# amazon-science/glass-text-spotting

Measured on AMD Instinct MI355X. Metric: images/sec/GPU end-to-end spotting, 1000x1000, ~32 RoIs; 1/2/4/8 GPU scaling, higher is better.
Workload: dtype f32

## Files before the change

glass-text-spotting_amd/csrc/wino_common.h:

```cpp
#pragma once
#include "common.h"
#include <cstdint>
#include <cstdlib>
#include <type_traits>
#include <utility>

typedef float f32x16 __attribute__((ext_vector_type(16)));
typedef unsigned u32x4 __attribute__((ext_vector_type(4)));

namespace {

constexpr unsigned OOB = 0x7fffffffu;

struct WinoParams {
  const float* x;
  const float* u;
  const float* bias;
  const float* res;
  float* y;
  int N, H, W, Cin, Cout, TH, TW, ntiles, nk;
  int nkt;
  long y_slice;
  int ldx, ldy, ycoff, ldr, relu, res_mode;
  int tiles_m, tiles_n;
  unsigned x_bytes, u_bytes, y_bytes, r_bytes;
  unsigned magic_tpi, magic_tw;
  unsigned long long* dbg;
};

__device__ __forceinline__ float4 add4(float4 a, float4 b) { return make_float4(a.x + b.x, a.y + b.y, a.z + b.z, a.w + b.w); }
__device__ __forceinline__ float4 sub4(float4 a, float4 b) { return make_float4(a.x - b.x, a.y - b.y, a.z - b.z, a.w - b.w); }
__device__ __forceinline__ int fast_div(int t, int d, unsigned magic) {
  int q = d == 1 ? t : (int)__umulhi((unsigned)t, magic);
  if (t - q * d >= d) ++q;
  return q;
}

template <int I> using ic = std::integral_constant<int, I>;
template <int... Is, class F> __device__ __forceinline__ void static_for_impl(std::integer_sequence<int, Is...>, F&& f) {
  (f(ic<Is>{}), ...);
}
template <int N, class F> __device__ __forceinline__ void static_for(F&& f) {
  static_for_impl(std::make_integer_sequence<int, N>{}, static_cast<F&&>(f));
}

__device__ __forceinline__ float comp(const float4& v, int s) { return s == 0 ? v.x : s == 1 ? v.y : s == 2 ? v.z : v.w; }

}
```

glass-text-spotting_amd/csrc/winograd43.hip:

```cpp
#include "wino_common.h"
#include "splitk_common.h"
#include <vector>

typedef float f32x4 __attribute__((ext_vector_type(4)));
typedef float f32x2 __attribute__((ext_vector_type(2)));
typedef unsigned u32x2 __attribute__((ext_vector_type(2)));

namespace {

constexpr int WINO43_LDS_BYTES = 2 * 36 * 16 * 32 * 4;
#ifndef GLASS_W43_RING
#define GLASS_W43_RING 6
#endif
constexpr int RING = GLASS_W43_RING;
#ifndef GLASS_W43_VACC_XI
#define GLASS_W43_VACC_XI 32
#endif
#ifndef GLASS_W43_STORE_AUX
#define GLASS_W43_STORE_AUX 0
#endif
constexpr int W43_STORE_AUX = GLASS_W43_STORE_AUX;
constexpr int VACC_XI = GLASS_W43_VACC_XI;
constexpr unsigned INV = 0x40000000u;

// ... 46 lines not shown
  constexpr int K4 = KT;
  constexpr int V4_FLOATS = 36 * T4 * K4;
  constexpr int HALVES = KT / 16;
  constexpr int NG = 36 * HALVES;
  constexpr int SPG = 144 / NG;
  constexpr int SLOTS = KT / 4;
  constexpr int RPW = 64 / KT;
  static_assert(NG % RING == 0, "ring slot = group % RING must be consistent across k-tiles");
  extern __shared__ __attribute__((aligned(16))) float smem[];
  const int nblk = gridDim.x, bid = blockIdx.x;
  const int xcd = bid & 7, q8 = nblk >> 3, r8 = nblk & 7;
  const int logical = (xcd < r8 ? xcd * (q8 + 1) : r8 * (q8 + 1) + (xcd - r8) * q8) + (bid >> 3);
  const int tile_m = logical / p.tiles_n;
  const int tile_n = logical - tile_m * p.tiles_n;
  const int t0 = tile_m * T4, n0 = tile_n * N4;

  const int tid = threadIdx.x, lane = tid & 63;
  const int wv = __builtin_amdgcn_readfirstlane(tid >> 6);
  const int tpi = p.TH * p.TW;
  const int kt0 = blockIdx.y * p.nk;
  const int xk0 = kt0 * (KT * 4), uk0 = tile_n * p.nkt + kt0;
  unsigned long long stamp0 = 0, stamp1 = 0, stamp2 = 0, real0 = 0;
  if constexpr (ABL == 4) { stamp0 = __builtin_amdgcn_s_memtime(); real0 = __builtin_amdgcn_s_memrealtime(); }

  __amdgpu_buffer_rsrc_t xr = __builtin_amdgcn_make_buffer_rsrc(const_cast<float*>(p.x), 0, (int)p.x_bytes, 0x00020000);
  __amdgpu_buffer_rsrc_t ur = __builtin_amdgcn_make_buffer_rsrc(const_cast<float*>(p.u), 0, (int)p.u_bytes, 0x00020000);

  const int c2 = tid % (KT / 2), tl = tid / (KT / 2);
  const int wc = WC == 4 ? wv : (wv & (WC - 1)), wt = WC == 4 ? 0 : (wv / WC);
  unsigned rowoff[6], coloff[6];
  {
    const int t = t0 + tl;
    const bool tv = t < p.ntiles;
    const int n = fast_div(t, tpi, p.magic_tpi);
    const int rem = t - n * tpi;
    const int th = fast_div(rem, p.TW, p.magic_tw);
    const int tw = rem - th * p.TW;
    const int h0 = 4 * th - 1, w0 = 4 * tw - 1;
#pragma unroll
    for (int r = 0; r < 6; ++r) {
      const int hi = h0 + r;
      rowoff[r] = (tv && (unsigned)hi < (unsigned)p.H) ? (unsigned)(((n * p.H + hi) * p.W) * p.ldx * 4) : INV;
    }
#pragma unroll
    for (int c = 0; c < 6; ++c) {
      const int wi = w0 + c;
      coloff[c] = ((unsigned)wi < (unsigned)p.W) ? (unsigned)((wi * p.ldx + 2 * c2) * 4) : INV;
    }
  }
  f32x2 dd[36];
  auto load_patch1 = [&](int kt, auto i_) {
    constexpr int i = decltype(i_)::value;
    if constexpr (ABL == 3) { if (kt > 1) return; }
    dd[i] = __builtin_bit_cast(f32x2, __builtin_amdgcn_raw_buffer_load_b64(xr, rowoff[i / 6] + coloff[i % 6], xk0 + kt * (K4 * 4), 0));
  };
  float* vdst = smem + tl * K4 + (((c2 >> 1) ^ ((tl / RPW) % SLOTS)) * 4) + (c2 & 1) * 2;
  Bt6p bt;
  auto row_step = [&](auto c_, auto s_) {
    constexpr int c = decltype(c_)::value, S = decltype(s_)::value;
    if constexpr (ABL == 2) return;
    bt.template step<S>(dd[0 + c], dd[6 + c], dd[12 + c], dd[18 + c], dd[24 + c], dd[30 + c]);
    if constexpr (S == 5) {
      dd[0 + c] = bt.o0; dd[6 + c] = bt.o1; dd[12 + c] = bt.o2; dd[18 + c] = bt.o3; dd[24 + c] = bt.o4; dd[30 + c] = bt.o5;
    }
  };
  auto vstore = [&](int stage, int xi, f32x2 v) {
    *reinterpret_cast<f32x2*>(vdst + stage * V4_FLOATS + xi * (T4 * K4)) = v;
  };
  auto col_step = [&](int stage, auto i_, auto s_) {
    constexpr int i = decltype(i_)::value, S = decltype(s_)::value;
    if constexpr (ABL == 2) {
      if constexpr (S == 1) vstore(stage, i * 6 + 0, dd[i * 6 + 0]);
      if constexpr (S == 2) vstore(stage, i * 6 + 1, dd[i * 6 + 1]);
      if constexpr (S == 3) vstore(stage, i * 6 + 2, dd[i * 6 + 2]);
      if constexpr (S == 4) vstore(stage, i * 6 + 5, dd[i * 6 + 5]);
      if constexpr (S == 5) { vstore(stage, i * 6 + 3, dd[i * 6 + 3]); vstore(stage, i * 6 + 4, dd[i * 6 + 4]); }
      return;
    }
    bt.template step<S>(dd[i * 6 + 0], dd[i * 6 + 1], dd[i * 6 + 2], dd[i * 6 + 3], dd[i * 6 + 4], dd[i * 6 + 5]);
    if constexpr (S == 1) vstore(stage, i * 6 + 0, bt.o0);
// ... 74 lines not shown
        }
        if constexpr (xi >= VACC_XI) {
          f32x4 c = acc[xi][cb];
          const float af = comp4(aq[u % RING][cb], s), bf = comp4(vq[u & 1], s);
          asm volatile("v_mfma_f32_16x16x4_f32 %0, %1, %2, %0" : "+v"(c) : "v"(af), "v"(bf));
          acc[xi][cb] = c;
        } else {
          acc[xi][cb] = __builtin_amdgcn_mfma_f32_16x16x4f32(comp4(aq[u % RING][cb], s), comp4(vq[u & 1], s), acc[xi][cb], 0, 0, 0);
        }
      });
      __builtin_amdgcn_sched_barrier(0);
    });
    __syncthreads();
  }

  if constexpr (VACC_XI < 36) {
    asm volatile("s_nop 15\n\ts_nop 15" ::: "memory");
#pragma unroll
    for (int i = VACC_XI; i < 36; ++i) {
      asm volatile("" : "+v"(acc[i][0]));
      asm volatile("" : "+v"(acc[i][1]));
    }
  }
  if constexpr (ABL == 4) stamp2 = __builtin_amdgcn_s_memtime();
  __amdgpu_buffer_rsrc_t yr = __builtin_amdgcn_make_buffer_rsrc(p.y + (long)blockIdx.y * p.y_slice, 0, (int)p.y_bytes, 0x00020000);
  __amdgpu_buffer_rsrc_t rr = __builtin_amdgcn_make_buffer_rsrc(const_cast<float*>(p.res_mode == 1 ? p.res : p.y), 0,
                                                                 (int)(p.res_mode == 1 ? p.r_bytes : 0u), 0x00020000);
  const int cbase = n0 + 32 * wc + 4 * kg;
  const unsigned ldy4 = (unsigned)p.ldy * 4u, ldr4 = (unsigned)p.ldr * 4u;
  unsigned yrow[4], ycol[4], rrow[4], rcol[4];
  {
    const int t = t0 + vt;
    const bool tv = t < p.ntiles;
    const int n = fast_div(t, tpi, p.magic_tpi);
    const int rem = t - n * tpi;
    const int th = fast_div(rem, p.TW, p.magic_tw);
    const int tw = rem - th * p.TW;
    const unsigned pix = (unsigned)((n * p.H + 4 * th) * p.W + 4 * tw);
#pragma unroll
    for (int a = 0; a < 4; ++a) {
      const bool ok = tv && 4 * th + a < p.H;
      yrow[a] = ok ? (pix + (unsigned)(a * p.W)) * ldy4 + (unsigned)(p.ycoff + cbase) * 4u : INV;
      rrow[a] = ok ? (pix + (unsigned)(a * p.W)) * ldr4 + (unsigned)cbase * 4u : INV;
    }
#pragma unroll
    for (int b = 0; b < 4; ++b) {
      const bool ok = 4 * tw + b < p.W;
      ycol[b] = ok ? (unsigned)b * ldy4 : INV;
      rcol[b] = ok ? (unsigned)b * ldr4 : INV;
    }
  }
  const float lo2 = p.relu == 2 ? 0.f : __builtin_nanf(""), lo1 = p.relu == 1 ? 0.f : __builtin_nanf("");
  f32x4 rres[2][16];
  auto load_res = [&](auto cb_) {
    constexpr int cb = decltype(cb_)::value;
    if (p.res_mode == 1) {
#pragma unroll
      for (int a = 0; a < 4; ++a)
#pragma unroll
        for (int b = 0; b < 4; ++b)
          rres[cb][a * 4 + b] = __builtin_bit_cast(f32x4, __builtin_amdgcn_raw_buffer_load_b128(rr, rrow[a] + rcol[b], cb * 64, 0));
    }
  };
#ifdef GLASS_W43_SPLIT_STORES
  load_res(ic<0>{});
  static_for<2>([&](auto cb_) {
    constexpr int cb = decltype(cb_)::value;
    f32x4 bv = f32x4{0.f, 0.f, 0.f, 0.f};
    if (p.bias != nullptr) bv = *reinterpret_cast<const f32x4*>(p.bias + cbase + 16 * cb);
    f32x4 out[16];
#pragma unroll
    for (int e = 0; e < 4; ++e) {
      float z[6][4];
#pragma unroll
      for (int i = 0; i < 6; ++i)
        at4(acc[i * 6 + 0][cb][e], acc[i * 6 + 1][cb][e], acc[i * 6 + 2][cb][e], acc[i * 6 + 3][cb][e], acc[i * 6 + 4][cb][e],
            acc[i * 6 + 5][cb][e], z[i][0], z[i][1], z[i][2], z[i][3]);
#pragma unroll
      for (int b = 0; b < 4; ++b) {
        float y0, y1, y2, y3;
        at4(z[0][b], z[1][b], z[2][b], z[3][b], z[4][b], z[5][b], y0, y1, y2, y3);
        out[0 * 4 + b][e] = y0; out[1 * 4 + b][e] = y1; out[2 * 4 + b][e] = y2; out[3 * 4 + b][e] = y3;
// ... 97 lines not shown
}

}

static bool wino43_wide(int Cout, int Cin) { return Cout % 128 == 0 && Cin % 32 == 0; }

extern "C" int glass_winograd43_supported(const glass_conv_desc* d) {
  if (!d) return 0;
  const long xb = (long)d->N * d->H * d->W * d->ldx * 4;
  const long yb = (long)d->N * d->H * d->W * d->ldy * 4, rb = d->res_mode == 1 ? (long)d->N * d->H * d->W * d->ldr * 4 : 0;
  const long lim = 0x40000000L;
  return d->KH == 3 && d->KW == 3 && d->stride_h == 1 && d->stride_w == 1 && d->pad_h == 1 && d->pad_w == 1 &&
         d->Cin % 16 == 0 && d->Cout % 64 == 0 && d->ldx % 2 == 0 && d->ldx >= d->Cin && d->y_cstride == 1 && d->ldy % 4 == 0 &&
         d->y_coff % 4 == 0 && d->y_coff >= 0 && d->y_coff + d->Cout <= d->ldy &&
         (d->res_mode == 0 || (d->res_mode == 1 && d->ldr % 4 == 0 && d->ldr >= d->Cout)) && xb < lim && yb < lim && rb < lim &&
         36L * d->Cout * d->Cin * 4 < 0x7fffff00L && d->Ho == d->H && d->Wo == d->W;
}

extern "C" size_t glass_winograd43_weight_floats(int Cout, int Cin) { return (size_t)36 * (size_t)Cout * (size_t)Cin; }

extern "C" int glass_winograd43_pack_weights(const float* w, int Cout, int Cin, float* u_packed, glass_stream_t stream) {
  GLASS_CHECK_ARG(w && u_packed, "glass_winograd43_pack_weights: null pointer");
  GLASS_CHECK_ARG(Cout > 0 && Cin > 0 && Cout % 64 == 0 && Cin % 16 == 0,
                  "glass_winograd43_pack_weights: Cout=%d must be a multiple of 64 and Cin=%d a multiple of 16", Cout, Cin);
  const long total = 36L * Cout * Cin;
  const int blocks = (int)((total + 255) / 256 < 8192 ? (total + 255) / 256 : 8192);
  const bool wide = wino43_wide(Cout, Cin);
  hipLaunchKernelGGL(wino43_pack_weights_kernel, dim3(blocks), dim3(256), 0, (hipStream_t)stream, w, u_packed, Cout, Cin,
                     wide ? 4 : 2, wide ? 32 : 16);
  GLASS_CHECK_LAUNCH("glass_winograd43_pack_weights");
  return GLASS_OK;
}

static int wino43_launch(const glass_conv_desc* d, const float* x, const float* u_packed, const float* bias, const float* residual,
                         float* y, glass_stream_t stream, bool body_only, int splits = 1, void* workspace = nullptr);

extern "C" int glass_conv3x3_winograd43_nhwc(const glass_conv_desc* d, const float* x, const float* u_packed,
                                             const float* bias, const float* residual, float* y, glass_stream_t stream) {
  return wino43_launch(d, x, u_packed, bias, residual, y, stream, false);
}

extern "C" int glass_conv3x3_winograd43_body_nhwc(const glass_conv_desc* d, const float* x, const float* u_packed,
                                                  const float* bias, const float* residual, float* y, glass_stream_t stream) {
  GLASS_CHECK_ARG(d && d->W >= 4, "glass_conv3x3_winograd43_body_nhwc: needs W >= 4");
  return wino43_launch(d, x, u_packed, bias, residual, y, stream, true);
}

extern "C" int glass_winograd43_splitk_supported(const glass_conv_desc* d, int splits) {
  return glass_winograd43_supported(d) && wino43_wide(d->Cout, d->Cin) && splits >= 2 && splits <= 32 && (d->Cin / 32) % splits == 0 &&
         (long)d->N * d->H * d->W * d->Cout * 4 < 0x40000000L;
}

extern "C" int64_t glass_winograd43_splitk_workspace_bytes(const glass_conv_desc* d, int splits) {
  if (!d) return 0;
  return (int64_t)splits * d->N * d->H * d->W * d->Cout * (int64_t)sizeof(float);
}

extern "C" int glass_conv3x3_winograd43_splitk_nhwc(const glass_conv_desc* d, const float* x, const float* u_packed, const float* bias,
                                                    const float* residual, float* y, int splits, int body_only, void* workspace,
                                                    int64_t workspace_bytes, glass_stream_t stream) {
  GLASS_CHECK_ARG(d && workspace, "glass_conv3x3_winograd43_splitk_nhwc: null pointer");
  GLASS_CHECK_ARG(glass_winograd43_splitk_supported(d, splits),
                  "glass_conv3x3_winograd43_splitk_nhwc: needs the wide F(4x4) shape (Cout %% 128 == 0, Cin %% 32 == 0), 2 <= splits <= 32 "
                  "dividing Cin / 32 (got Cin=%d Cout=%d splits=%d)", d->Cin, d->Cout, splits);
  GLASS_CHECK_ARG(workspace_bytes >= glass_winograd43_splitk_workspace_bytes(d, splits) && ((uintptr_t)workspace & 15) == 0,
                  "glass_conv3x3_winograd43_splitk_nhwc: workspace too small or not 16-byte aligned");
  GLASS_CHECK_ARG(!body_only || d->W >= 4, "glass_conv3x3_winograd43_splitk_nhwc: body_only needs W >= 4");
  return wino43_launch(d, x, u_packed, bias, residual, y, stream, body_only != 0, splits, workspace);
}

static int wino43_launch(const glass_conv_desc* d, const float* x, const float* u_packed, const float* bias, const float* residual,
                         float* y, glass_stream_t stream, bool body_only, int splits, void* workspace) {
  GLASS_CHECK_ARG(d && x && u_packed && y, "glass_conv3x3_winograd43_nhwc: null pointer");
  GLASS_CHECK_ARG(glass_winograd43_supported(d),
                  "glass_conv3x3_winograd43_nhwc: needs 3x3/stride 1/pad 1, Cin%%16==0, Cout%%64==0, unit channel stride, "
                  "res_mode 0/1 and operands < 1 GiB (got Cin=%d Cout=%d k=%dx%d s=%d p=%d)", d->Cin, d->Cout, d->KH, d->KW,
                  d->stride_h, d->pad_h);
  GLASS_CHECK_ARG(d->res_mode == 0 || residual != nullptr, "glass_conv3x3_winograd43_nhwc: res_mode set but residual is null");
  GLASS_CHECK_ARG(((uintptr_t)x & 15) == 0 && ((uintptr_t)u_packed & 15) == 0 && ((uintptr_t)y & 15) == 0 &&
                      (bias == nullptr || ((uintptr_t)bias & 15) == 0) && (residual == nullptr || ((uintptr_t)residual & 15) == 0),
                  "glass_conv3x3_winograd43_nhwc: pointers must be 16-byte aligned");
  if (d->N == 0) return GLASS_OK;
  WinoParams p;
  p.x = x; p.u = u_packed; p.bias = bias; p.res = residual; p.y = y; p.dbg = nullptr;
  p.N = d->N; p.H = d->H; p.W = d->W; p.Cin = d->Cin; p.Cout = d->Cout;
  p.TH = (d->H + 3) / 4; p.TW = body_only ? d->W / 4 : (d->W + 3) / 4;
  const long nt = (long)d->N * p.TH * p.TW;
  GLASS_CHECK_ARG(nt < 0x7fffffffL, "glass_conv3x3_winograd43_nhwc: too many tiles");
  p.ntiles = (int)nt;
  const bool wide = wino43_wide(d->Cout, d->Cin);
  const int T4 = wide ? 16 : 32, N4 = wide ? 128 : 64, K4 = wide ? 32 : 16;
  p.nkt = d->Cin / K4;
  p.nk = p.nkt / splits;
  p.y_slice = 0;
  p.ldx = d->ldx; p.ldy = d->ldy; p.ycoff = d->y_coff; p.ldr = d->ldr; p.relu = d->relu; p.res_mode = d->res_mode;
  p.tiles_m = cdiv(p.ntiles, T4);
  p.tiles_n = d->Cout / N4;
  p.x_bytes = (unsigned)((long)d->N * d->H * d->W * d->ldx * 4);
  p.magic_tpi = (unsigned)(0x100000000ULL / (unsigned long long)(p.TH * p.TW));
  p.magic_tw = (unsigned)(0x100000000ULL / (unsigned long long)p.TW);
  p.u_bytes = (unsigned)(36L * d->Cout * d->Cin * 4);
  p.y_bytes = (unsigned)((long)d->N * d->H * d->W * d->ldy * 4);
  p.r_bytes = d->res_mode == 1 ? (unsigned)((long)d->N * d->H * d->W * d->ldr * 4) : 0u;
  const long Mpix = (long)d->N * d->H * d->W;
  if (splits > 1) {
    p.y = static_cast<float*>(workspace); p.bias = nullptr; p.res = nullptr;
    p.ldy = d->Cout; p.ycoff = 0; p.relu = 0; p.res_mode = 0; p.ldr = 0; p.r_bytes = 0;
    p.y_slice = Mpix * d->Cout;
    p.y_bytes = (unsigned)(Mpix * d->Cout * 4);
  }
  const long nblk = (long)p.tiles_m * p.tiles_n;
  GLASS_CHECK_ARG(nblk > 0 && nblk <= 0x7fffffffL, "glass_conv3x3_winograd43_nhwc: bad grid");
  static const int abl = getenv("GLASS_W43_ABL") ? atoi(getenv("GLASS_W43_ABL")) : 0;
  auto kern = !wide ? (abl == 4 ? conv3x3_wino43_f32<4, 2, 2, 16> : conv3x3_wino43_f32<0, 2, 2, 16>)
#ifdef GLASS_W43_ABLATIONS
            : abl == 1 ? conv3x3_wino43_f32<1, 1, 4, 32> : abl == 2 ? conv3x3_wino43_f32<2, 1, 4, 32> : abl == 3 ? conv3x3_wino43_f32<3, 1, 4, 32>
#endif
            : abl == 4 ? conv3x3_wino43_f32<4, 1, 4, 32> : conv3x3_wino43_f32<0, 1, 4, 32>;
  static unsigned long long* dbg_dev = nullptr;
  if (abl == 4) {
    if (!dbg_dev) (void)hipMalloc(&dbg_dev, 8L * 8 * 65536);
    p.dbg = nblk <= 65536 ? dbg_dev : nullptr;
// ... 45 lines not shown
```

glass-text-spotting_amd/glass_amd/_lib.py:

```python
from __future__ import annotations

import ctypes
import glob
import os
import subprocess
from typing import List, Optional

_PKG = os.path.dirname(os.path.abspath(__file__))
_ROOT = os.path.dirname(_PKG)
CSRC = os.path.join(_ROOT, "csrc")
INCLUDE = os.path.join(os.path.dirname(_ROOT), "include")
SO_PATH = os.environ.get("GLASS_HIP_LIB") or os.path.join(_ROOT, "libglass_hip.so")

EXPORTS = [
    "glass_last_error", "glass_abi_version", "glass_device_count", "glass_conv2d_nhwc", "glass_conv2d_nhwc_f16", "glass_conv2d_nhwc_h16", "glass_local_stem_supported", "glass_local_stem_fused", "glass_local_stem_fused_h16", "glass_backbone_stem_supported", "glass_backbone_stem_fused", "glass_conv3x3_winograd43_body_nhwc", "glass_winograd43_splitk_supported", "glass_winograd43_splitk_workspace_bytes", "glass_conv3x3_winograd43_splitk_nhwc", "glass_roi_align_rotated_up2", "glass_conv2d_splitk_supported", "glass_conv2d_splitk_workspace_bytes", "glass_conv2d_nhwc_splitk", "glass_conv3x3_winograd_body_nhwc",
    "glass_pointwise_supported", "glass_pointwise_weight_floats", "glass_pointwise_pack_weights", "glass_conv1x1_pointwise_nhwc",
    "glass_pointwise_split_supported", "glass_pointwise_split_weight_bytes", "glass_pointwise_split_pack_weights", "glass_conv1x1_pointwise_split_nhwc", "glass_pointwise_split_dual_supported", "glass_conv1x1_pointwise_split_dual_nhwc",
    "glass_conv_h16_supported", "glass_conv_h16_weight_halves", "glass_conv_h16_pack_weights", "glass_conv2d_nhwc_h16_packed",
    "glass_winograd_supported", "glass_winograd_block_channels", "glass_winograd_weight_floats", "glass_winograd_pack_weights", "glass_conv3x3_winograd_nhwc",
    "glass_winograd43_supported", "glass_winograd43_weight_floats", "glass_winograd43_pack_weights", "glass_conv3x3_winograd43_nhwc",
    "glass_maxpool2d_nhwc", "glass_maxpool2d_nhwc_h16", "glass_roi_align_rotated_h16", "glass_pixel_shuffle2x_nhwc", "glass_sigmoid_inplace", "glass_paste_rotated_masks", "glass_mul_inplace", "glass_cast_f32_to_f16",
    "glass_preprocess_image", "glass_image_u8hwc_to_chw_resized", "glass_roi_align_rotated",
    "glass_rpn_workspace_bytes", "glass_rpn_topk_decode", "glass_rotated_nms_select", "glass_pairwise_iou_rotated", "glass_detections_finalize", "glass_postprocess_words", "glass_postprocess_words_dense_workspace_bytes", "glass_postprocess_words_dense", "glass_text_argmax", "glass_pack_word_records",
    "glass_box_decode", "glass_gc_attention_inplace", "glass_mean_over_h", "glass_bilstm_workspace_bytes", "glass_bilstm_recurrence",
    "glass_bilstm_persistent_workspace_bytes", "glass_bilstm_recurrence_persistent", "glass_recurrence_status", "glass_recurrence_test_hook",
    "glass_decode_persistent_supported", "glass_decode_persistent_workspace_bytes", "glass_attention_decode_persistent",
    "glass_decode_workspace_bytes", "glass_attention_decode", "glass_decode_step_workspace_bytes", "glass_attention_decode_step",
    "glass_lexicon_match_workspace_bytes", "glass_lexicon_match",
    "glass_lexicon_match_weighted_workspace_bytes", "glass_lexicon_match_weighted",
    "glass_rrc_pair_areas_workspace_bytes", "glass_rrc_pair_areas", "glass_rrc_match_workspace_bytes", "glass_rrc_match",
    "glass_rrc_sweep_workspace_bytes", "glass_rrc_sweep",
    "glass_mask_windows", "glass_mask_rings_workspace_bytes", "glass_mask_rings_count", "glass_mask_rings_write",
    "glass_ring_check_tasks", "glass_ring_check",
]


class GlassLibraryError(RuntimeError):
    pass


DEVICE_FLAGS = ["-Xclang", "-target-feature", "-Xclang", "-packed-fp32-ops", "-Xclang", "-target-feature", "-Xclang", "-fma-mix-insts"]


ABI_VERSION = 8


def sources() -> List[str]:
    return sorted(glob.glob(os.path.join(CSRC, "*.hip")))


def source_sha16() -> str:
    import hashlib
    h = hashlib.sha256()
# ... 87 lines not shown
```

glass-text-spotting_amd/glass_amd/ops/native.py:

```python
from __future__ import annotations

import collections
import ctypes
import math
import os
import struct
import threading
from typing import List, NamedTuple, Optional, Sequence, Tuple

import numpy as np
import torch

from .._lib import GlassLibraryError, check, lib

c_int, c_float, c_void_p = ctypes.c_int, ctypes.c_float, ctypes.c_void_p


class ConvDesc(ctypes.Structure):
    _fields_ = [(n, c_int) for n in (
        "N", "H", "W", "Cin", "Cout", "KH", "KW", "stride_h", "stride_w", "pad_h", "pad_w", "Ho", "Wo",
        "ldx", "ldy", "y_coff", "y_cstride", "relu", "res_mode", "ldr")]


class RoiAlignDesc(ctypes.Structure):
# ... 46 lines not shown
    sh, sw = _pair(stride)
    ph, pw = _pair(padding)
    return (H + 2 * ph - KH) // sh + 1, (W + 2 * pw - KW) // sw + 1


_PRECISIONS = ("fp32", "fp16", "fp16s")


_RNN_LAYOUTS = ((1, 1), (2, 1), (2, 2))


def _parse_rnn(v):
    if isinstance(v, str) and v in ("steps", "persistent"):
        return v
    try:
        nd, ng = (int(t) for t in (v if isinstance(v, (tuple, list)) else str(v).split("x")))
    except (TypeError, ValueError):
        nd = ng = -1
    if (nd, ng) not in _RNN_LAYOUTS:
        raise GlassLibraryError(f"unknown recurrent routing {v!r} (steps | persistent | 2x1 | 2x2 | 1x1)")
    return (nd, ng)


def _parse_split(v) -> int:
    try:
        n = int(v)
    except (TypeError, ValueError):
        n = -1
    if n not in (0, 6, 9):
        raise GlassLibraryError(f"unknown 1x1 split routing {v!r} (0 | 9 | 6)")
    return n


class Routing:
    __slots__ = ("precision", "winograd", "f43", "pw", "h16", "local_stem", "stem", "ragged", "pooled_fusion", "rnn", "splitk", "small_grid", "split")

    def __init__(self, precision: Optional[str] = None, winograd: Optional[bool] = None, f43: Optional[bool] = None, pw=None,
                 h16: Optional[bool] = None, local_stem: Optional[bool] = None, stem: Optional[bool] = None,
                 ragged: Optional[bool] = None, pooled_fusion: Optional[bool] = None, rnn=None,
                 splitk: Optional[bool] = None, small_grid: Optional[bool] = None, split: Optional[int] = None):
        e = os.environ.get
        self.precision = precision or e("GLASS_CONV_PRECISION", "fp32")
        if self.precision not in _PRECISIONS:
            raise GlassLibraryError(f"unknown conv precision {self.precision!r}")
        self.winograd = (e("GLASS_WINOGRAD", "1") != "0") if winograd is None else bool(winograd)
        self.f43 = (e("GLASS_WINOGRAD43", "1") != "0") if f43 is None else bool(f43)
        self.pw = {"0": False, "all": "all"}.get(e("GLASS_POINTWISE", "1"), True) if pw is None else (pw if pw == "all" else bool(pw))
        self.h16 = (e("GLASS_CONV_H16", "1") != "0") if h16 is None else bool(h16)
        self.local_stem = (e("GLASS_LOCAL_STEM", "1") != "0") if local_stem is None else bool(local_stem)
        self.stem = (e("GLASS_BACKBONE_STEM", "1") != "0") if stem is None else bool(stem)
        self.ragged = (e("GLASS_W43_RAGGED", "1") != "0") if ragged is None else bool(ragged)
        self.pooled_fusion = (e("GLASS_POOLED_FUSION", "1") != "0") if pooled_fusion is None else bool(pooled_fusion)
        self.rnn = _parse_rnn(e("GLASS_RNN", "1x1")) if rnn is None else _parse_rnn(rnn)
        self.splitk = (e("GLASS_SPLITK", "1") != "0") if splitk is None else bool(splitk)
        self.small_grid = (e("GLASS_SMALL_GRID", "1") != "0") if small_grid is None else bool(small_grid)
        self.split = _parse_split(e("GLASS_PW_SPLIT", "9") if split is None else split)

    def replace(self, **kw) -> "Routing":
        r = Routing.__new__(Routing)
        for k in Routing.__slots__:
            setattr(r, k, kw.pop(k, getattr(self, k)))
        if kw:
            raise TypeError(f"unknown routing fields {sorted(kw)}")
        if r.precision not in _PRECISIONS:
            raise GlassLibraryError(f"unknown conv precision {r.precision!r}")
        r.split = _parse_split(r.split)
        r.rnn = _parse_rnn(r.rnn)
        return r

    @property
    def act_dtype(self) -> torch.dtype:
        return torch.float16 if self.precision == "fp16s" else torch.float32

    def __repr__(self):
        return "Routing(" + ", ".join(f"{k}={getattr(self, k)!r}" for k in Routing.__slots__) + ")"


_DEFAULT = Routing()
_TLS = threading.local()
_COUNTS = {"on_the_fly": 0}


def default_routing() -> Routing:
    return _DEFAULT


def routing_of(w) -> Routing:
    r = getattr(w, "routing", None)
    return r if r is not None else _DEFAULT


def set_conv_precision(precision: str) -> str:
    if precision not in _PRECISIONS:
        raise GlassLibraryError(f"unknown conv precision {precision!r}")
    prev = _DEFAULT.precision
    _DEFAULT.precision = precision
    return prev


def conv_precision() -> str:
# ... 132 lines not shown

    @property
    def shape(self):
        return self.raw.shape

    @property
    def device(self):
        return self.raw.device

    def nbytes(self) -> int:
        return self.raw.numel() * 4 + sum(u.numel() * u.element_size() for u in self.packs.values())


class packing_for:

    def __init__(self, routing):
        self.routing = routing if isinstance(routing, Routing) else Routing(precision=routing)

    def __enter__(self):
        self.prev = getattr(_TLS, "load", None)
        _TLS.load = self.routing
        return self

    def __exit__(self, *exc):
        _TLS.load = self.prev
        return False


def _probe_desc(Cout: int, KH: int, KW: int, Cin: int) -> ConvDesc:
    ph, pw = KH // 2, KW // 2
    return ConvDesc(1, 16, 16, Cin, Cout, KH, KW, 1, 1, ph, pw, 16 + 2 * ph - KH + 1, 16 + 2 * pw - KW + 1, Cin, Cout, 0, 1, 0, 0, 0)


def pack_kinds(Cout: int, KH: int, KW: int, Cin: int, precision: str, stride=1, ragged: bool = False, split: int = 0) -> list:
    if precision == "all":
        return pack_kinds(Cout, KH, KW, Cin, "fp32", stride, ragged, split=9) + pack_kinds(Cout, KH, KW, Cin, "fp16", stride)
    L, d = lib(), _probe_desc(Cout, KH, KW, Cin)
    kinds = []
    if precision == "fp32":
        if KH == 3 and KW == 3 and _pair(stride) == (1, 1):
            if L.glass_winograd_supported(ctypes.byref(d)):
                kinds.append(False)
            if L.glass_winograd43_supported(ctypes.byref(d)):
                kinds.append(True)
                if ragged and (2 * Cin) % 32 == 0:
                    kinds.append("col1")
        if KH == 1 and KW == 1 and L.glass_pointwise_supported(ctypes.byref(d)):
            kinds.append("pw")
        if split and KH == 1 and KW == 1 and L.glass_pointwise_split_supported(ctypes.byref(d)):
            kinds.append("pws")
    elif Cin % 64 == 0 and L.glass_conv_h16_supported(ctypes.byref(d), 1):
        kinds.append("h16")
    return kinds


def prepare_conv_weights(w: torch.Tensor, precision: Optional[str] = None, stride=1, ragged: bool = False) -> ConvWeight:
    if isinstance(w, ConvWeight):
        return w
    if w.dim() == 2:
        w = w.view(w.shape[0], 1, 1, w.shape[1])
    load = getattr(_TLS, "load", None)
    cw = ConvWeight(w, routing=load)
    precision = precision or (load.precision if load is not None else _DEFAULT.precision)
    Cout, KH, KW, Cin = w.shape
    if w.is_cuda:
        for kind in pack_kinds(Cout, KH, KW, Cin, precision, stride, ragged, split=(load.split if load is not None else _DEFAULT.split)):
            cw.packs[kind] = winograd_pack(w, kind)
        if cw.packs and load is None:
            torch.cuda.current_stream().synchronize()
    return cw


def packs_on_the_fly() -> int:
    return _COUNTS["on_the_fly"]


def _packed(w, wt: torch.Tensor, kind) -> torch.Tensor:
    if isinstance(w, ConvWeight):
        if w.version is not None and not wt.is_inference() and w.version != wt._version:
            for k in list(w.packs):
                w.packs[k] = winograd_pack(wt, k)
            w.version = wt._version
            _COUNTS["on_the_fly"] += 1
        u = w.packs.get(kind)
        if u is not None:
            return u
    _COUNTS["on_the_fly"] += 1
    return winograd_pack(wt, kind)


class ConvPlan(NamedTuple):
    path: str
    entry: str
    pack: object = None
    flags: Optional[int] = None
    splits: int = 0
    strip: bool = False
    cast: bool = False

# ... 7 lines not shown
              res_mode: int, packs, forced=None, f43k=None) -> ConvPlan:
    L, dp = lib(), ctypes.byref(d)
    N, H, W, Cin, Cout, KH, KW, sh, sw, _, _, Ho, Wo, ldx, _, _, y_cstride, _, _, _ = _DESC_INTS.unpack(d)
    three = KH == 3 and KW == 3
    half = (1 if x_dtype == torch.float16 else 0) | (2 if out_dtype == torch.float16 else 0) | (4 if res_dtype == torch.float16 else 0)
    if half:
        if rt.precision != "fp16s" or forced:
            raise GlassLibraryError("float16 activation tensors need conv precision 'fp16s' (and no forced Winograd)")
        if rt.h16 and L.glass_conv_h16_supported(dp, half):
            return ConvPlan("packed_fp16", "glass_conv2d_nhwc_h16_packed", "h16", half)
        return ConvPlan("direct_fp16", "glass_conv2d_nhwc_h16", None, half)
    if rt.precision in ("fp16", "fp16s") and not forced:
        if rt.h16 and KH * KW * Cout >= 512 and N * H * W * ldx > 0 and L.glass_conv_h16_supported(dp, 1):
            return ConvPlan("packed_fp16", "glass_conv2d_nhwc_h16_packed", "h16", 1, cast=True)
        return ConvPlan("direct_fp16", "glass_conv2d_nhwc_f16")
    px = N * Ho * Wo
    if forced in ("pws9", "pws6"):
        if not L.glass_pointwise_split_supported(dp):
            raise GlassLibraryError(f"winograd={forced!r} but glass_pointwise_split_supported() rejects this layer")
        return ConvPlan("pointwise_split", "glass_conv1x1_pointwise_split_nhwc", "pws", int(forced[3]))
    auto_1x1 = forced is None and KH == 1 and KW == 1
    if (auto_1x1 and rt.split and _use_split(px, Cin, Cout) and L.glass_pointwise_split_supported(dp) and
            (packs is None or "pws" in packs)):
        return ConvPlan("pointwise_split", "glass_conv1x1_pointwise_split_nhwc", "pws", rt.split)
    if (auto_1x1 and rt.pw and
            (rt.pw == "all" or (Cin >= 256 and Cout >= 256 and px >= 16384) or (Cin >= 512 and Cout >= 512 and px >= 8192))
            and L.glass_pointwise_supported(dp)):
        return ConvPlan("pointwise", "glass_conv1x1_pointwise_nhwc", "pw")
    use_wino = rt.winograd if forced is None else forced
    if forced is None and use_wino and three:
        use_wino = ((N * ((H + 1) // 2) * ((W + 1) // 2) + 63) // 64) * (Cout // 64) >= 96
    can_strip = (rt.ragged and three and W % 2 == 1 and W >= 5 and (2 * Cin) % 32 == 0 and y_cstride == 1 and ldx == Cin and
                 res_mode in (0, 1) and N * H * W * ldx > 0 and (packs is None or "col1" in packs))
    ragged = can_body = can_strip and W % 4 == 1
    f43 = forced == "f43" or (forced is None and rt.f43 and use_wino and three and _use_f43(N, H, W, Cout, Cin, ragged))
    f22_body = forced == "f22r"
    if f22_body and not can_strip:
        raise GlassLibraryError("winograd='f22r' needs an odd width >= 5, dense input, unit channel stride and res_mode 0/1")
    t_alt = None
    if forced is None and use_wino and not f43 and three and rt.small_grid and L.glass_winograd_supported(dp):
        kind, body, t_alt = _small_grid_3x3(N, H, W, Cout, Cin, can_strip, rt.f43 and bool(L.glass_winograd43_supported(dp)))
        f43, ragged, f22_body = kind == "f43", kind == "f43" and body, kind == "f22" and body
    if (forced is None and rt.winograd and rt.f43 and rt.small_grid and rt.splitk and rt.precision == "fp32" and three and
            sh == 1 and sw == 1 and out_dtype == torch.float32 and y_cstride == 1 and res_mode in (0, 1) and
            not _use_f43(N, H, W, Cout, Cin, can_body) and (packs is None or True in packs)):
        plan = _f43_splitk_plan(N, H, W, Cout, Cin, can_strip)
        if f43k is not None:
            sl, body = f43k if isinstance(f43k, tuple) else (f43k, False)
            plan, t_alt = ((int(sl), bool(body) and can_body, 0.0) if sl else None), None
        if plan is not None:
            sl, body, t_sk = plan
            if t_alt is None and not use_wino:
                t_alt = _splitk_slices(rt, px, KH * KW * Cin, Cin, Cout, want_time=True)[1]
            if (t_alt is None or t_sk < (0.8 if body else 0.85) * t_alt) and L.glass_winograd43_splitk_supported(dp, sl):
                return ConvPlan("winograd43k", "glass_conv3x3_winograd43_splitk_nhwc", True, int(body), sl, strip=body)
    if use_wino and f43 and three and L.glass_winograd43_supported(dp):
        if ragged:
            return ConvPlan("winograd43r", "glass_conv3x3_winograd43_body_nhwc", True, strip=True)
        return ConvPlan("winograd43", "glass_conv3x3_winograd43_nhwc", True)
    if forced == "f43":
        raise GlassLibraryError("winograd='f43' but glass_winograd43_supported() rejects this layer")
    if use_wino and three and L.glass_winograd_supported(dp):
        path = "winograd128" if L.glass_winograd_block_channels(Cout, Cin) == 128 else "winograd"
        if f22_body:
            return ConvPlan(path + "r", "glass_conv3x3_winograd_body_nhwc", False, strip=True)
        return ConvPlan(path, "glass_conv3x3_winograd_nhwc", False)
    if forced:
        raise GlassLibraryError("winograd=True but glass_winograd_supported() rejects this layer")
    splits = _splitk_slices(rt, px, KH * KW * Cin, Cin, Cout) if (res_mode in (0, 1) or res_dtype is None) else 0
    if splits > 1 and out_dtype == torch.float32 and L.glass_conv2d_splitk_supported(dp, splits):
        return ConvPlan("direct", "glass_conv2d_nhwc_splitk", splits=splits)
    return ConvPlan("direct", "glass_conv2d_nhwc")


def conv2d_nhwc(x: torch.Tensor, w, bias: Optional[torch.Tensor] = None, *, stride=1, padding=0,
                relu: int = 0, residual: Optional[torch.Tensor] = None, res_mode: int = 0,
                out: Optional[torch.Tensor] = None, out_coff: int = 0, out_cstride: int = 1,
                cin: Optional[int] = None, winograd: Optional[bool] = None, out_dtype: Optional[torch.dtype] = None,
                precision: Optional[str] = None, routing: Optional[Routing] = None, f43k=None) -> torch.Tensor:
    wt = w.raw if isinstance(w, ConvWeight) else _f32c(w, "w")
    rt = routing if routing is not None else routing_of(w)
    if precision is not None and precision != rt.precision:
        rt = rt.replace(precision=precision)
    _fhc(x, "x")
    N, H, W, ldx = x.shape
    Cout, KH, KW, Cin = wt.shape
    if cin is not None and cin != Cin:
        raise GlassLibraryError(f"cin={cin} does not match weight Cin={Cin}")
    sh, sw = _pair(stride)
# ... 928 lines not shown
```

include/glass_hip.h:

```cpp
#ifndef GLASS_HIP_H
#define GLASS_HIP_H

#include <stddef.h>
#include <stdint.h>

#ifdef __cplusplus
extern "C" {
#endif

#define GLASS_OK 0
#define GLASS_EINVAL (-1)
#define GLASS_EHIP (-2)
#define GLASS_ENOMEM (-3)

typedef void* glass_stream_t;

const char* glass_last_error(void);
int glass_abi_version(void);
int glass_device_count(void);

typedef struct glass_conv_desc {
  int N, H, W, Cin;
  int Cout, KH, KW;
  int stride_h, stride_w, pad_h, pad_w;
// ... 4 lines not shown
  int res_mode;
  int ldr;
} glass_conv_desc;

int glass_conv2d_nhwc(const glass_conv_desc* d, const float* x, const float* w, const float* bias,
                      const float* residual, float* y, glass_stream_t stream);

int glass_conv2d_nhwc_f16(const glass_conv_desc* d, const float* x, const float* w, const float* bias,
                          const float* residual, float* y, glass_stream_t stream);

int glass_conv2d_nhwc_h16(const glass_conv_desc* d, const void* x, const float* w, const float* bias, const void* residual,
                          void* y, int flags, glass_stream_t stream);

int glass_conv_h16_supported(const glass_conv_desc* d, int flags);
size_t glass_conv_h16_weight_halves(int Cout, int KH, int KW, int Cin);
int glass_conv_h16_pack_weights(const float* w, int Cout, int KH, int KW, int Cin, void* u_packed, glass_stream_t stream);
int glass_conv2d_nhwc_h16_packed(const glass_conv_desc* d, const void* x, const void* u_packed, const float* bias,
                                 const void* residual, void* y, int flags, glass_stream_t stream);

int glass_winograd_supported(const glass_conv_desc* d);
int glass_winograd_block_channels(int Cout, int Cin);
size_t glass_winograd_weight_floats(int Cout, int Cin);
int glass_winograd_pack_weights(const float* w, int Cout, int Cin, float* u_packed, glass_stream_t stream);
int glass_conv3x3_winograd_nhwc(const glass_conv_desc* d, const float* x, const float* u_packed, const float* bias,
                                const float* residual, float* y, glass_stream_t stream);

int glass_winograd43_supported(const glass_conv_desc* d);
size_t glass_winograd43_weight_floats(int Cout, int Cin);
int glass_winograd43_pack_weights(const float* w, int Cout, int Cin, float* u_packed, glass_stream_t stream);
int glass_conv3x3_winograd43_nhwc(const glass_conv_desc* d, const float* x, const float* u_packed, const float* bias,
                                  const float* residual, float* y, glass_stream_t stream);
int glass_conv3x3_winograd43_body_nhwc(const glass_conv_desc* d, const float* x, const float* u_packed, const float* bias,
                                       const float* residual, float* y, glass_stream_t stream);
int glass_winograd43_splitk_supported(const glass_conv_desc* d, int splits);
int64_t glass_winograd43_splitk_workspace_bytes(const glass_conv_desc* d, int splits);
int glass_conv3x3_winograd43_splitk_nhwc(const glass_conv_desc* d, const float* x, const float* u_packed, const float* bias,
                                         const float* residual, float* y, int splits, int body_only, void* workspace,
                                         int64_t workspace_bytes, glass_stream_t stream);
int glass_conv3x3_winograd_body_nhwc(const glass_conv_desc* d, const float* x, const float* u_packed, const float* bias,
                                     const float* residual, float* y, glass_stream_t stream);

int glass_pointwise_supported(const glass_conv_desc* d);
size_t glass_pointwise_weight_floats(int Cout, int Cin);
int glass_pointwise_pack_weights(const float* w, int Cout, int Cin, float* u_packed, glass_stream_t stream);
int glass_conv1x1_pointwise_nhwc(const glass_conv_desc* d, const float* x, const float* u_packed, const float* bias,
                                 const float* residual, float* y, glass_stream_t stream);

int glass_pointwise_split_supported(const glass_conv_desc* d);
size_t glass_pointwise_split_weight_bytes(int Cout, int Cin);
int glass_pointwise_split_pack_weights(const float* w, int Cout, int Cin, void* u_packed, glass_stream_t stream);
int glass_conv1x1_pointwise_split_nhwc(const glass_conv_desc* d, const float* x, const void* u_packed, const float* bias,
                                       const float* residual, float* y, int products, glass_stream_t stream);
int glass_pointwise_split_dual_supported(const glass_conv_desc* d, int Cin2, int ldx2);
int glass_conv1x1_pointwise_split_dual_nhwc(const glass_conv_desc* d, const float* x1, const float* x2, int Cin2, int ldx2,
                                            const void* u_packed, const float* bias, float* y, glass_stream_t stream);

int glass_local_stem_supported(int H, int W);
int glass_local_stem_fused(const float* x, const float* w1, const float* b1, const float* w2, const float* b2, float* y,
                           int R, int H, int W, glass_stream_t stream);
int glass_local_stem_fused_h16(const float* x, const float* w1, const float* b1, const float* w2, const float* b2, void* y,
                               int R, int H, int W, glass_stream_t stream);

int glass_conv2d_splitk_supported(const glass_conv_desc* d, int splits);
int64_t glass_conv2d_splitk_workspace_bytes(const glass_conv_desc* d, int splits);
int glass_conv2d_nhwc_splitk(const glass_conv_desc* d, const float* x, const float* w, const float* bias, const float* residual,
                             float* y, int splits, void* workspace, int64_t workspace_bytes, glass_stream_t stream);
// ... 179 lines not shown
```

Before: 312.4.

## Handle ragged last column in Winograd F(4,3) kernel via paired-image strip tiles

For layers with W = 4k+1, the Winograd F(4,3) kernel gains extra tiles that cover the leftover last column by packing two images' edge columns side by side into a single 4-wide tile. This replaces the separate body-plus-strip path, which needed an extra col1 weight pack and a second kernel launch. The new tiles waste part of the transform on padding and add index math per tile. Routing defaults to the new mode, and the strip weight packs are now skipped unless they are needed.

```diff
diff --git a/glass-text-spotting_amd/csrc/wino_common.h b/glass-text-spotting_amd/csrc/wino_common.h
--- a/glass-text-spotting_amd/csrc/wino_common.h
+++ b/glass-text-spotting_amd/csrc/wino_common.h
@@ -26,6 +26,8 @@
   unsigned x_bytes, u_bytes, y_bytes, r_bytes;
   unsigned magic_tpi, magic_tw;
   unsigned long long* dbg;
+  int nbody;
+  unsigned magic_th;
 };
 
 __device__ __forceinline__ float4 add4(float4 a, float4 b) { return make_float4(a.x + b.x, a.y + b.y, a.z + b.z, a.w + b.w); }
diff --git a/glass-text-spotting_amd/csrc/winograd43.hip b/glass-text-spotting_amd/csrc/winograd43.hip
--- a/glass-text-spotting_amd/csrc/winograd43.hip
+++ b/glass-text-spotting_amd/csrc/winograd43.hip
@@ -102,11 +102,17 @@
   {
     const int t = t0 + tl;
     const bool tv = t < p.ntiles;
-    const int n = fast_div(t, tpi, p.magic_tpi);
-    const int rem = t - n * tpi;
-    const int th = fast_div(rem, p.TW, p.magic_tw);
-    const int tw = rem - th * p.TW;
+    const bool st = t >= p.nbody;
+    const int s = t - p.nbody;
+    const int sq = fast_div(s, p.TH, p.magic_th);
+    const int sth = s - sq * p.TH;
+    const int nb = fast_div(t, tpi, p.magic_tpi);
+    const int rem = t - nb * tpi;
+    const int thb = fast_div(rem, p.TW, p.magic_tw);
+    const int tw = rem - thb * p.TW;
+    const int n = st ? 2 * sq : nb, th = st ? sth : thb;
     const int h0 = 4 * th - 1, w0 = 4 * tw - 1;
+    const bool hasb = n + 1 < p.N;
 #pragma unroll
     for (int r = 0; r < 6; ++r) {
       const int hi = h0 + r;
@@ -114,8 +120,8 @@
     }
 #pragma unroll
     for (int c = 0; c < 6; ++c) {
-      const int wi = w0 + c;
-      coloff[c] = ((unsigned)wi < (unsigned)p.W) ? (unsigned)((wi * p.ldx + 2 * c2) * 4) : INV;
+      const int wi = st ? (c % 3 == 2 || (c >= 3 && !hasb) ? -1 : (c >= 3 ? p.H * p.W : 0) + p.W - 2 + c % 3) : w0 + c;
+      coloff[c] = ((unsigned)wi < (unsigned)(st ? 2 * p.H * p.W : p.W)) ? (unsigned)((wi * p.ldx + 2 * c2) * 4) : INV;
     }
   }
   f32x2 dd[36];
@@ -256,11 +262,17 @@
   {
     const int t = t0 + vt;
     const bool tv = t < p.ntiles;
-    const int n = fast_div(t, tpi, p.magic_tpi);
-    const int rem = t - n * tpi;
-    const int th = fast_div(rem, p.TW, p.magic_tw);
-    const int tw = rem - th * p.TW;
-    const unsigned pix = (unsigned)((n * p.H + 4 * th) * p.W + 4 * tw);
+    const bool st = t >= p.nbody;
+    const int s = t - p.nbody;
+    const int sq = fast_div(s, p.TH, p.magic_th);
+    const int sth = s - sq * p.TH;
+    const int nb = fast_div(t, tpi, p.magic_tpi);
+    const int rem = t - nb * tpi;
+    const int thb = fast_div(rem, p.TW, p.magic_tw);
+    const int tw = rem - thb * p.TW;
+    const int n = st ? 2 * sq : nb, th = st ? sth : thb;
+    const unsigned pix = (unsigned)((n * p.H + 4 * th) * p.W + (st ? p.W - 1 : 4 * tw));
+    const unsigned img = (unsigned)(p.H * p.W);
 #pragma unroll
     for (int a = 0; a < 4; ++a) {
       const bool ok = tv && 4 * th + a < p.H;
@@ -269,9 +281,10 @@
     }
 #pragma unroll
     for (int b = 0; b < 4; ++b) {
-      const bool ok = 4 * tw + b < p.W;
-      ycol[b] = ok ? (unsigned)b * ldy4 : INV;
-      rcol[b] = ok ? (unsigned)b * ldr4 : INV;
+      const bool ok = st ? (b == 0 || (b == 3 && n + 1 < p.N)) : 4 * tw + b < p.W;
+      const unsigned pb = st ? (b == 3 ? img : 0u) : (unsigned)b;
+      ycol[b] = ok ? pb * ldy4 : INV;
+      rcol[b] = ok ? pb * ldr4 : INV;
     }
   }
   const float lo2 = p.relu == 2 ? 0.f : __builtin_nanf(""), lo1 = p.relu == 1 ? 0.f : __builtin_nanf("");
@@ -435,18 +448,34 @@
   return GLASS_OK;
 }
 
+enum { W43_FULL = 0, W43_BODY = 1, W43_RAGGED = 2 };
 static int wino43_launch(const glass_conv_desc* d, const float* x, const float* u_packed, const float* bias, const float* residual,
-                         float* y, glass_stream_t stream, bool body_only, int splits = 1, void* workspace = nullptr);
+                         float* y, glass_stream_t stream, int mode, int splits = 1, void* workspace = nullptr);
 
 extern "C" int glass_conv3x3_winograd43_nhwc(const glass_conv_desc* d, const float* x, const float* u_packed,
                                              const float* bias, const float* residual, float* y, glass_stream_t stream) {
-  return wino43_launch(d, x, u_packed, bias, residual, y, stream, false);
+  return wino43_launch(d, x, u_packed, bias, residual, y, stream, W43_FULL);
 }
 
 extern "C" int glass_conv3x3_winograd43_body_nhwc(const glass_conv_desc* d, const float* x, const float* u_packed,
                                                   const float* bias, const float* residual, float* y, glass_stream_t stream) {
   GLASS_CHECK_ARG(d && d->W >= 4, "glass_conv3x3_winograd43_body_nhwc: needs W >= 4");
-  return wino43_launch(d, x, u_packed, bias, residual, y, stream, true);
+  return wino43_launch(d, x, u_packed, bias, residual, y, stream, W43_BODY);
+}
+
+extern "C" int glass_winograd43_ragged_supported(const glass_conv_desc* d) {
+  if (!glass_winograd43_supported(d) || d->W % 4 != 1 || d->W < 5) return 0;
+  const long img = (long)d->H * d->W * 4, lim = 0x40000000L;
+  return ((long)d->N + 1) * img * d->ldx < lim && ((long)d->N + 1) * img * d->ldy < lim &&
+         (d->res_mode != 1 || ((long)d->N + 1) * img * d->ldr < lim);
+}
+
+extern "C" int glass_conv3x3_winograd43_ragged_nhwc(const glass_conv_desc* d, const float* x, const float* u_packed,
+                                                    const float* bias, const float* residual, float* y, glass_stream_t stream) {
+  GLASS_CHECK_ARG(d && glass_winograd43_ragged_supported(d),
+                  "glass_conv3x3_winograd43_ragged_nhwc: needs a layer glass_winograd43_supported() takes, W = 4 k + 1 >= 5 and operands "
+                  "+ one image < 1 GiB (got W=%d)", d ? d->W : 0);
+  return wino43_launch(d, x, u_packed, bias, residual, y, stream, W43_RAGGED);
 }
 
 extern "C" int glass_winograd43_splitk_supported(const glass_conv_desc* d, int splits) {
@@ -469,11 +498,11 @@
   GLASS_CHECK_ARG(workspace_bytes >= glass_winograd43_splitk_workspace_bytes(d, splits) && ((uintptr_t)workspace & 15) == 0,
                   "glass_conv3x3_winograd43_splitk_nhwc: workspace too small or not 16-byte aligned");
   GLASS_CHECK_ARG(!body_only || d->W >= 4, "glass_conv3x3_winograd43_splitk_nhwc: body_only needs W >= 4");
-  return wino43_launch(d, x, u_packed, bias, residual, y, stream, body_only != 0, splits, workspace);
+  return wino43_launch(d, x, u_packed, bias, residual, y, stream, body_only != 0 ? W43_BODY : W43_FULL, splits, workspace);
 }
 
 static int wino43_launch(const glass_conv_desc* d, const float* x, const float* u_packed, const float* bias, const float* residual,
-                         float* y, glass_stream_t stream, bool body_only, int splits, void* workspace) {
+                         float* y, glass_stream_t stream, int mode, int splits, void* workspace) {
   GLASS_CHECK_ARG(d && x && u_packed && y, "glass_conv3x3_winograd43_nhwc: null pointer");
   GLASS_CHECK_ARG(glass_winograd43_supported(d),
                   "glass_conv3x3_winograd43_nhwc: needs 3x3/stride 1/pad 1, Cin%%16==0, Cout%%64==0, unit channel stride, "
@@ -487,10 +516,13 @@
   WinoParams p;
   p.x = x; p.u = u_packed; p.bias = bias; p.res = residual; p.y = y; p.dbg = nullptr;
   p.N = d->N; p.H = d->H; p.W = d->W; p.Cin = d->Cin; p.Cout = d->Cout;
-  p.TH = (d->H + 3) / 4; p.TW = body_only ? d->W / 4 : (d->W + 3) / 4;
-  const long nt = (long)d->N * p.TH * p.TW;
+  p.TH = (d->H + 3) / 4; p.TW = mode != W43_FULL ? d->W / 4 : (d->W + 3) / 4;
+  const long nbody = (long)d->N * p.TH * p.TW;
+  const long nt = nbody + (mode == W43_RAGGED ? ((long)d->N + 1) / 2 * p.TH : 0);
   GLASS_CHECK_ARG(nt < 0x7fffffffL, "glass_conv3x3_winograd43_nhwc: too many tiles");
   p.ntiles = (int)nt;
+  p.nbody = mode == W43_RAGGED ? (int)nbody : p.ntiles;
+  p.magic_th = (unsigned)(0x100000000ULL / (unsigned long long)p.TH);
   const bool wide = wino43_wide(d->Cout, d->Cin);
   const int T4 = wide ? 16 : 32, N4 = wide ? 128 : 64, K4 = wide ? 32 : 16;
   p.nkt = d->Cin / K4;
diff --git a/glass-text-spotting_amd/glass_amd/_lib.py b/glass-text-spotting_amd/glass_amd/_lib.py
--- a/glass-text-spotting_amd/glass_amd/_lib.py
+++ b/glass-text-spotting_amd/glass_amd/_lib.py
@@ -19,6 +19,7 @@
     "glass_conv_h16_supported", "glass_conv_h16_weight_halves", "glass_conv_h16_pack_weights", "glass_conv2d_nhwc_h16_packed",
     "glass_winograd_supported", "glass_winograd_block_channels", "glass_winograd_weight_floats", "glass_winograd_pack_weights", "glass_conv3x3_winograd_nhwc",
     "glass_winograd43_supported", "glass_winograd43_weight_floats", "glass_winograd43_pack_weights", "glass_conv3x3_winograd43_nhwc",
+    "glass_winograd43_ragged_supported", "glass_conv3x3_winograd43_ragged_nhwc",
     "glass_maxpool2d_nhwc", "glass_maxpool2d_nhwc_h16", "glass_roi_align_rotated_h16", "glass_pixel_shuffle2x_nhwc", "glass_sigmoid_inplace", "glass_paste_rotated_masks", "glass_mul_inplace", "glass_cast_f32_to_f16",
     "glass_preprocess_image", "glass_image_u8hwc_to_chw_resized", "glass_roi_align_rotated",
     "glass_rpn_workspace_bytes", "glass_rpn_topk_decode", "glass_rotated_nms_select", "glass_pairwise_iou_rotated", "glass_detections_finalize", "glass_postprocess_words", "glass_postprocess_words_dense_workspace_bytes", "glass_postprocess_words_dense", "glass_text_argmax", "glass_pack_word_records",
diff --git a/glass-text-spotting_amd/glass_amd/ops/native.py b/glass-text-spotting_amd/glass_amd/ops/native.py
--- a/glass-text-spotting_amd/glass_amd/ops/native.py
+++ b/glass-text-spotting_amd/glass_amd/ops/native.py
@@ -102,12 +102,18 @@
     return n
 
 
+def _parse_ragged(v):
+    if isinstance(v, str):
+        return {"0": False, "strip": True}.get(v, "tiles")
+    return bool(v)
+
+
 class Routing:
     __slots__ = ("precision", "winograd", "f43", "pw", "h16", "local_stem", "stem", "ragged", "pooled_fusion", "rnn", "splitk", "small_grid", "split")
 
     def __init__(self, precision: Optional[str] = None, winograd: Optional[bool] = None, f43: Optional[bool] = None, pw=None,
                  h16: Optional[bool] = None, local_stem: Optional[bool] = None, stem: Optional[bool] = None,
-                 ragged: Optional[bool] = None, pooled_fusion: Optional[bool] = None, rnn=None,
+                 ragged=None, pooled_fusion: Optional[bool] = None, rnn=None,
                  splitk: Optional[bool] = None, small_grid: Optional[bool] = None, split: Optional[int] = None):
         e = os.environ.get
         self.precision = precision or e("GLASS_CONV_PRECISION", "fp32")
@@ -119,7 +125,7 @@
         self.h16 = (e("GLASS_CONV_H16", "1") != "0") if h16 is None else bool(h16)
         self.local_stem = (e("GLASS_LOCAL_STEM", "1") != "0") if local_stem is None else bool(local_stem)
         self.stem = (e("GLASS_BACKBONE_STEM", "1") != "0") if stem is None else bool(stem)
-        self.ragged = (e("GLASS_W43_RAGGED", "1") != "0") if ragged is None else bool(ragged)
+        self.ragged = _parse_ragged(e("GLASS_W43_RAGGED", "tiles") if ragged is None else ragged)
         self.pooled_fusion = (e("GLASS_POOLED_FUSION", "1") != "0") if pooled_fusion is None else bool(pooled_fusion)
         self.rnn = _parse_rnn(e("GLASS_RNN", "1x1")) if rnn is None else _parse_rnn(rnn)
         self.splitk = (e("GLASS_SPLITK", "1") != "0") if splitk is None else bool(splitk)
@@ -136,6 +142,7 @@
             raise GlassLibraryError(f"unknown conv precision {r.precision!r}")
         r.split = _parse_split(r.split)
         r.rnn = _parse_rnn(r.rnn)
+        r.ragged = _parse_ragged(r.ragged)
         return r
 
     @property
@@ -334,7 +341,8 @@
     return ConvDesc(1, 16, 16, Cin, Cout, KH, KW, 1, 1, ph, pw, 16 + 2 * ph - KH + 1, 16 + 2 * pw - KW + 1, Cin, Cout, 0, 1, 0, 0, 0)
 
 
-def pack_kinds(Cout: int, KH: int, KW: int, Cin: int, precision: str, stride=1, ragged: bool = False, split: int = 0) -> list:
+def pack_kinds(Cout: int, KH: int, KW: int, Cin: int, precision: str, stride=1, ragged: bool = False, split: int = 0,
+               strip: bool = True) -> list:
     if precision == "all":
         return pack_kinds(Cout, KH, KW, Cin, "fp32", stride, ragged, split=9) + pack_kinds(Cout, KH, KW, Cin, "fp16", stride)
     L, d = lib(), _probe_desc(Cout, KH, KW, Cin)
@@ -345,7 +353,7 @@
                 kinds.append(False)
             if L.glass_winograd43_supported(ctypes.byref(d)):
                 kinds.append(True)
-                if ragged and (2 * Cin) % 32 == 0:
+                if ragged and strip and (2 * Cin) % 32 == 0:
                     kinds.append("col1")
         if KH == 1 and KW == 1 and L.glass_pointwise_supported(ctypes.byref(d)):
             kinds.append("pw")
@@ -354,6 +362,10 @@
     elif Cin % 64 == 0 and L.glass_conv_h16_supported(ctypes.byref(d), 1):
         kinds.append("h16")
     return kinds
+
+
+def needs_strip_pack(rt: Routing) -> bool:
+    return bool(rt.ragged and rt.winograd and (rt.small_grid or rt.ragged != "tiles"))
 
 
 def prepare_conv_weights(w: torch.Tensor, precision: Optional[str] = None, stride=1, ragged: bool = False) -> ConvWeight:
@@ -366,7 +378,8 @@
     precision = precision or (load.precision if load is not None else _DEFAULT.precision)
     Cout, KH, KW, Cin = w.shape
     if w.is_cuda:
-        for kind in pack_kinds(Cout, KH, KW, Cin, precision, stride, ragged, split=(load.split if load is not None else _DEFAULT.split)):
+        rt = load if load is not None else _DEFAULT
+        for kind in pack_kinds(Cout, KH, KW, Cin, precision, stride, ragged, split=rt.split, strip=needs_strip_pack(rt)):
             cw.packs[kind] = winograd_pack(w, kind)
         if cw.packs and load is None:
             torch.cuda.current_stream().synchronize()
@@ -440,7 +453,10 @@
         use_wino = ((N * ((H + 1) // 2) * ((W + 1) // 2) + 63) // 64) * (Cout // 64) >= 96
     can_strip = (rt.ragged and three and W % 2 == 1 and W >= 5 and (2 * Cin) % 32 == 0 and y_cstride == 1 and ldx == Cin and
                  res_mode in (0, 1) and N * H * W * ldx > 0 and (packs is None or "col1" in packs))
-    ragged = can_body = can_strip and W % 4 == 1
+    can_body = can_strip and W % 4 == 1
+    can_ragged = (rt.ragged == "tiles" and three and W % 4 == 1 and y_cstride == 1 and res_mode in (0, 1) and N * H * W * ldx > 0 and
+                  bool(L.glass_winograd43_ragged_supported(dp)))
+    ragged = can_ragged or can_body
     f43 = forced == "f43" or (forced is None and rt.f43 and use_wino and three and _use_f43(N, H, W, Cout, Cin, ragged))
     f22_body = forced == "f22r"
     if f22_body and not can_strip:
@@ -463,6 +479,8 @@
             if (t_alt is None or t_sk < (0.8 if body else 0.85) * t_alt) and L.glass_winograd43_splitk_supported(dp, sl):
                 return ConvPlan("winograd43k", "glass_conv3x3_winograd43_splitk_nhwc", True, int(body), sl, strip=body)
     if use_wino and f43 and three and L.glass_winograd43_supported(dp):
+        if ragged and can_ragged:
+            return ConvPlan("winograd43r", "glass_conv3x3_winograd43_ragged_nhwc", True)
         if ragged:
             return ConvPlan("winograd43r", "glass_conv3x3_winograd43_body_nhwc", True, strip=True)
         return ConvPlan("winograd43", "glass_conv3x3_winograd43_nhwc", True)
diff --git a/include/glass_hip.h b/include/glass_hip.h
--- a/include/glass_hip.h
+++ b/include/glass_hip.h
@@ -60,6 +60,9 @@
                                   const float* residual, float* y, glass_stream_t stream);
 int glass_conv3x3_winograd43_body_nhwc(const glass_conv_desc* d, const float* x, const float* u_packed, const float* bias,
                                        const float* residual, float* y, glass_stream_t stream);
+int glass_winograd43_ragged_supported(const glass_conv_desc* d);
+int glass_conv3x3_winograd43_ragged_nhwc(const glass_conv_desc* d, const float* x, const float* u_packed, const float* bias,
+                                         const float* residual, float* y, glass_stream_t stream);
 int glass_winograd43_splitk_supported(const glass_conv_desc* d, int splits);
 int64_t glass_winograd43_splitk_workspace_bytes(const glass_conv_desc* d, int splits);
 int glass_conv3x3_winograd43_splitk_nhwc(const glass_conv_desc* d, const float* x, const float* u_packed, const float* bias,
```

Result: faster. 316.4 (median of 6 runs) (+1.3%).
